# gaurav00700/Selfsupervised-NVSF

Hardware: AMD Instinct MI355X
Metric: rendered rays/sec (LiDAR+cam) (higher is better)
Workload: dtype f16; 1 GPU; C2: KITTI-360 seq-1908-shaped frame per GPU, uniform sampling, static hash field; num_rays=4096, num_rays_lidar=4096, num_steps=768, hash_grid=L16 F2 T2^19 base16 max2048, sigma_mlp=32-64-16, heads=lidar 2x(87-64-64-1), rgb 31-64-64-3, parallelism=frame-sharded x1, no collective

## Files before the change

selfsupervised-nvsf_amd/csrc/common.h:

```cpp
#pragma once
#include <hip/hip_runtime.h>
#include <stdint.h>

#define NVSF_API extern "C" __attribute__((visibility("default")))

enum : int {
    NVSF_OK = 0,
    NVSF_ERR_INVALID_ARG = -1,
    NVSF_ERR_UNSUPPORTED = -2,
};

constexpr int kWave = 64;

static inline int nvsf_launch_status() {
    hipError_t e = hipGetLastError();
    return e == hipSuccess ? NVSF_OK : (int)e;
}

static inline unsigned cdiv(unsigned long long a, unsigned b) { return (unsigned)((a + b - 1) / b); }

enum NvsfVariantKey : int {
    kVarMarch = 0,
    kVarPlanesFwd,
    kVarPlanesBwd,
    kVarHashgridFwd,
    kVarHashgridBwd,
    kVarHash4dBwd,
    kVarSlicePlan,
    kVarRenderTail,
    kVarMarchSkew,
    kVarMlpBwd,
    kVarLevelKinds,
    kVarCount
};
int nvsf_variant(int key);
int nvsf_cu_count();

__device__ __forceinline__ int lane_id() { return (int)(threadIdx.x & 63); }

template <typename T>
__device__ __forceinline__ T wave_sum(T v) {
#pragma unroll
    for (int o = 32; o > 0; o >>= 1) v += __shfl_xor(v, o, 64);
    return v;
}

__device__ __forceinline__ float wave_scan_add(float v) {
    const int l = lane_id();
#pragma unroll
    for (int o = 1; o < 64; o <<= 1) {
        float u = __shfl_up(v, o, 64);
        if (l >= o) v += u;
    }
    return v;
}
__device__ __forceinline__ float wave_scan_mul(float v) {
    const int l = lane_id();
#pragma unroll
    for (int o = 1; o < 64; o <<= 1) {
        float u = __shfl_up(v, o, 64);
        if (l >= o) v *= u;
    }
    return v;
}
__device__ __forceinline__ uint32_t wave_scan_add_u32(uint32_t v) {
// ... 25 lines not shown
```

selfsupervised-nvsf_amd/csrc/fused_field.hip:

```cpp
#include "hashgrid_device.h"
#include "mlp_device.h"
#include "encodings_device.h"
#include "march_device.h"
#pragma clang diagnostic ignored "-Wpass-failed"
#include <stdlib.h>

namespace {
constexpr int kBlock = 256;
constexpr int kWavesPerBlock = kBlock / kWave;

struct RayBatch {
    const float* rays_o;
    const float* rays_d;
    const float* nears;
    const float* fars;
    const float* lin;
    const float* noise;
    float lo[3], hi[3];
    float inv_extent;
    float bound;
    uint32_t N, T;
};

template <int F>
// ... 68 lines not shown
__device__ __forceinline__ void fma_entry(float w, uint32_t raw, float& a0, float& a1) {
    asm("v_fma_mix_f32 %0, %1, %2, %0 op_sel_hi:[0,1,0]" : "+v"(a0) : "v"(w), "v"(raw));
    asm("v_fma_mix_f32 %0, %1, %2, %0 op_sel:[0,1,0] op_sel_hi:[0,1,0]" : "+v"(a1) : "v"(w), "v"(raw));
}

template <int F>
__device__ __forceinline__ uint32_t gather_raw(__amdgpu_buffer_rsrc_t rsrc, uint32_t byte_off);
template <>
__device__ __forceinline__ uint32_t gather_raw<2>(__amdgpu_buffer_rsrc_t rsrc, uint32_t byte_off) {
    return __builtin_amdgcn_raw_buffer_load_b32(rsrc, byte_off, 0, 0);
}
typedef uint32_t entry4_t __attribute__((ext_vector_type(2)));
template <int F> struct EntryOf { typedef uint32_t type; };
template <> struct EntryOf<4> { typedef entry4_t type; };
template <>
__device__ __forceinline__ uint32_t gather_raw<4>(__amdgpu_buffer_rsrc_t, uint32_t) = delete;
__device__ __forceinline__ entry4_t gather_raw4(__amdgpu_buffer_rsrc_t rsrc, uint32_t byte_off) {
    return __builtin_amdgcn_raw_buffer_load_b64(rsrc, byte_off, 0, 0);
}

template <int F>
struct DensityCtx {
    static constexpr int Q = 8 / F;
    LaneLevels<F> lv;
    half8_t w0[kHidTiles];
    OutLayerW wout;
    __amdgpu_buffer_rsrc_t rsrc;
    uint32_t first_hashed;
    int g;
    const uint4* lds_lv;
};

constexpr uint32_t kFirstHashedC2 = 5;
template <int F, int QG, bool LDS_LV = false, int FH = -1>
__device__ __forceinline__ half8_t density_encode(const DensityCtx<F>& cx, const float (&x)[3]) {
    constexpr int Q = 8 / F;
    LaneLevels<F> lv_local;
    if constexpr (LDS_LV) {
        uint32_t again = 0;
        asm volatile("" : "+v"(again));
#pragma unroll
        for (int q = 0; q < Q; ++q) {
            const uint4 v = cx.lds_lv[4 * q + again];
            lv_local.scale[q] = __builtin_bit_cast(float, v.x);
            lv_local.res[q] = v.y;
            lv_local.res2[q] = v.y * v.y;
            lv_local.boff[q] = v.z;
            lv_local.rows[q] = v.w;
        }
    }
    const LaneLevels<F>& lv = LDS_LV ? lv_local : cx.lv;
    const uint32_t first_hashed = FH >= 0 ? (uint32_t)FH : cx.first_hashed;
    const int g = cx.g;
    half8_t xf;
#pragma unroll
    for (int q0 = 0; q0 < Q; q0 += QG) {
    float frac[Q][3];
    typename EntryOf<F>::type raw[Q][8];
#pragma unroll
    for (int q = q0; q < q0 + QG; ++q) {
        uint32_t c[3];
#pragma unroll
        for (int d = 0; d < 3; ++d) {
            const float pos = fmaf(lv.scale[q], x[d], 0.5f);
            const float fl = floorf(pos);
            frac[q][d] = pos - fl;
            c[d] = (uint32_t)(int32_t)fl;
        }
        uint32_t idx[8];
        const bool all_dense = (uint32_t)(4 * q + 3) < first_hashed, all_hashed = (uint32_t)(4 * q) >= first_hashed;
        if (all_dense || !all_hashed) {
            const uint32_t b00 = c[0] + c[1] * lv.res[q] + c[2] * lv.res2[q];
            const uint32_t b10 = b00 + lv.res[q], b01 = b00 + lv.res2[q], b11 = b10 + lv.res2[q];
            const uint32_t base[4] = {b00, b10, b01, b11};
#pragma unroll
            for (int k = 0; k < 8; ++k) {
                uint32_t v = base[k >> 1] + (uint32_t)(k & 1);
                v = v >= lv.rows[q] ? v - lv.rows[q] : v;
                idx[k] = v;
            }
        }
        if (all_hashed || !all_dense) {
            const uint32_t hy0 = c[1] * 2654435761u, hy1 = hy0 + 2654435761u;
            const uint32_t hz0 = c[2] * 805459861u, hz1 = hz0 + 805459861u;
            const uint32_t yz[4] = {hy0 ^ hz0, hy1 ^ hz0, hy0 ^ hz1, hy1 ^ hz1};
            const uint32_t mask = lv.rows[q] - 1u;
            const bool lane_hashed = (uint32_t)(4 * q + g) >= first_hashed;
#pragma unroll
            for (int k = 0; k < 8; ++k) {
                const uint32_t v = ((c[0] + (uint32_t)(k & 1)) ^ yz[k >> 1]) & mask;
                idx[k] = (all_hashed || lane_hashed) ? v : idx[k];
            }
        }
#pragma unroll
        for (int k = 0; k < 8; ++k) {
            if constexpr (F == 2) raw[q][k] = gather_raw<2>(cx.rsrc, lv.boff[q] + idx[k] * (uint32_t)(F * sizeof(_Float16)));
            else raw[q][k] = gather_raw4(cx.rsrc, lv.boff[q] + idx[k] * (uint32_t)(F * sizeof(_Float16)));
        }
    }
#pragma unroll
    for (int q = q0; q < q0 + QG; ++q) {
        const float fx = frac[q][0], fy = frac[q][1], fz = frac[q][2];
        const float wx[2] = {1.0f - fx, fx}, wy[2] = {1.0f - fy, fy}, wz[2] = {1.0f - fz, fz};
        if constexpr (F == 2) {
            float a0 = 0.0f, a1 = 0.0f;
#pragma unroll
            for (int k = 0; k < 8; ++k) {
                const float w = (wx[k & 1] * wy[(k >> 1) & 1]) * wz[k >> 2];
                fma_entry(w, raw[q][k], a0, a1);
            }
            xf[q * F] = (_Float16)a0;
            xf[q * F + 1] = (_Float16)a1;
        } else {
            float a0 = 0.0f, a1 = 0.0f, a2 = 0.0f, a3 = 0.0f;
#pragma unroll
            for (int k = 0; k < 8; ++k) {
                const float w = (wx[k & 1] * wy[(k >> 1) & 1]) * wz[k >> 2];
                fma_entry(w, raw[q][k][0], a0, a1);
                fma_entry(w, raw[q][k][1], a2, a3);
            }
            xf[q * F] = (_Float16)a0;
            xf[q * F + 1] = (_Float16)a1;
            xf[q * F + 2] = (_Float16)a2;
            xf[q * F + 3] = (_Float16)a3;
        }
    }
    }
    return xf;
}

template <int F, int QG>
__device__ __forceinline__ float4_t density_eval(const DensityCtx<F>& cx, const float (&x)[3]) {
    const half8_t xf = density_encode<F, QG>(cx, x);
    float4_t acc1[kHidTiles];
#pragma unroll
    for (int t = 0; t < kHidTiles; ++t) {
        const float4_t zero = {0, 0, 0, 0};
        acc1[t] = mfma16(cx.w0[t], xf, zero);
    }
    half8_t h[kHidSteps];
    pack_hidden(acc1, h);
    return cx.wout.apply(h);
}

struct TrainOut {
    float* x01;
    _Float16* feat;
    float* h32;
    uint32_t* tile;
};

__device__ __forceinline__ void store_h32(float* __restrict__ h32, unsigned long long s, int lane, int g, float o0, float o1, float o2, float o3, bool ok) {
    const int from = (lane + 48) & 63;
    const float prev = __int_as_float(__builtin_amdgcn_ds_bpermute(from << 2, __float_as_int(o3)));
    if (ok) *reinterpret_cast<float4*>(h32 + s * 16 + 4 * g) = make_float4(prev, o0, o1, o2);
}

constexpr int kTrPitch = 20;
constexpr int kTrWords = 16 * kTrPitch;
// ... 1238 lines not shown
                    img[1] += w0 * cr[1];
                }
            } else {
                if (g == 0 && on) {
#pragma unroll
                    for (int k = 0; k < 3; ++k) {
                        cr[k] = sigmoid_f32(oa[k]);
                        img[k] += w0 * cr[k];
                    }
                }
            }
        }
        if constexpr (TRAIN) {
            if (g == 0 && valid) {
#pragma unroll
                for (int k = 0; k < C; ++k) rt.rgb[s * C + k] = cr[k];
            }
        }
    }
    ws = wave_sum(ws);
    dp = wave_sum(dp);
#pragma unroll
    for (int k = 0; k < C; ++k) img[k] = wave_sum(img[k]);
    if (lane == 0) {
        weights_sum[n] = ws;
        depth[n] = dp;
        const float bg[3] = {bg0, bg1, bg2};
        const float rest = use_bg ? 1.0f - ws : 0.0f;
#pragma unroll
        for (int k = 0; k < C; ++k) image[(size_t)n * C + k] = use_bg ? img[k] + rest * bg[k] : img[k];
    }
}

template <bool LIDAR, bool TRAIN = false>
__global__ __launch_bounds__(kBlock) __attribute__((amdgpu_waves_per_eu(4, 4))) void k_render_tail2(
    RayBatch rb, const uint2* __restrict__ feat, const _Float16* __restrict__ w_sigma, const _Float16* __restrict__ w_a,
    const _Float16* __restrict__ w_b, float k_scale, float w_thresh, float bg0, float bg1, float bg2, int use_bg,
    const float* __restrict__ z_vals, float* __restrict__ weights, float* __restrict__ weights_sum, float* __restrict__ depth,
    float* __restrict__ image, RenderTrainOut rt = RenderTrainOut()) {
    using FR = OccFrags<LIDAR>;
    constexpr int IN_STEPS = FR::IN_STEPS;
    constexpr int C = LIDAR ? 2 : 3;
    constexpr int kOut1 = FR::kCount;
    __shared__ half8_t s_frag[(FR::kCount + kHidSteps) * kWave];
    __shared__ float4_t s_pre[kWavesPerBlock * FR::kPre];
    const int lane = lane_id(), g = lane >> 4, c = lane & 15;
    for (int f = (int)(threadIdx.x >> 6); f < FR::kCount + kHidSteps; f += kWavesPerBlock)
        s_frag[f * kWave + lane] = f < FR::kCount ? occ_fragment<LIDAR>(f, lane, w_sigma, w_a, w_b) : load_w_chained(w_sigma + kHidden * 32, 0, f - FR::kCount, lane, 5);
    __syncthreads();
    const uint32_t n = __builtin_amdgcn_readfirstlane(blockIdx.x * kWavesPerBlock + (threadIdx.x >> 6));
    if (n >= rb.N) return;
    const half8_t* frag = s_frag + lane;
    const uint32_t T = rb.T;
    const size_t M = (size_t)rb.N * T;

    const float rd0 = rb.rays_d[3 * (size_t)n], rd1 = rb.rays_d[3 * (size_t)n + 1], rd2 = rb.rays_d[3 * (size_t)n + 2];
    const float d0 = (rd0 + 1.0f) / 2.0f, d1 = (rd1 + 1.0f) / 2.0f, d2 = (rd2 + 1.0f) / 2.0f;
    half8_t xf[IN_STEPS];
    if constexpr (!LIDAR) {
        float sh[16];
        sh4_basis(d0, d1, d2, sh);
#pragma unroll
        for (int j = 0; j < 8; ++j) xf[0][j] = (_Float16)(g == 0 ? sh[j] : sh[8 + j]);
    } else {
#pragma unroll
        for (int s = 0; s < 3; ++s)
#pragma unroll
            for (int j = 0; j < 8; j += 2) {
                const int k = 32 * s + 8 * g + j;
                float sn = 1.0f, cs = 1.0f;
                if (k < 72) {
                    const int i = k / 24, f = (k - 24 * i) >> 1;
                    freq_pair(i == 0 ? d0 : (i == 1 ? d1 : d2), f, sn, cs);
                }
                xf[s][j] = (_Float16)sn;
                xf[s][j + 1] = (_Float16)cs;
            }
    }
    const bool takes_geo = LIDAR ? (g == 1 || g == 2) : (g >= 2);
    const int src_a = (c + 16 * (LIDAR ? 2 * (g - 1) : 2 * (g - 2))) & 63, src_b = (src_a + 16) & 63;
    const int src_a1 = (src_a + 48) & 63, src_b1 = (src_b + 48) & 63;
    float4_t* pre = s_pre + (threadIdx.x >> 6) * FR::kPre;
    ray_head_constants<LIDAR>(xf, w_a, w_b, lane, pre);
    auto head2 = [&](int hd, const half8_t (&x_last)[2], float4_t (&out)[2]) {
        const int base = FR::kHead + hd * FR::kPerHead;
        float4_t acc[2][kHidTiles];
#pragma unroll
        for (int t = 0; t < kHidTiles; ++t) {
            float4_t c = {0, 0, 0, 0};
            if constexpr (IN_STEPS > 1) c = pre[(hd * 4 + t) * 4 + g];
            const half8_t w = frag[(base + t) * kWave];
            acc[0][t] = mfma16(w, x_last[0], c);
            acc[1][t] = mfma16(w, x_last[1], c);
        }
        half8_t h[2][kHidSteps];
        pack_hidden(acc[0], h[0]);
        pack_hidden(acc[1], h[1]);
#pragma unroll
        for (int t = 0; t < kHidTiles; ++t) {
            float4_t a0 = {0, 0, 0, 0}, a1 = {0, 0, 0, 0};
#pragma unroll
            for (int s = 0; s < kHidSteps; ++s) {
                const half8_t w = frag[(base + 4 + 2 * t + s) * kWave];
                a0 = mfma16(w, h[0][s], a0);
                a1 = mfma16(w, h[1][s], a1);
            }
            acc[0][t] = a0;
            acc[1][t] = a1;
        }
        pack_hidden(acc[0], h[0]);
        pack_hidden(acc[1], h[1]);
        float4_t a0 = {0, 0, 0, 0}, a1 = {0, 0, 0, 0};
#pragma unroll
        for (int s = 0; s < kHidSteps; ++s) {
            const half8_t w = frag[(base + 4 + 8 + s) * kWave];
            a0 = mfma16(w, h[0][s], a0);
            a1 = mfma16(w, h[1][s], a1);
        }
        out[0] = a0;
        out[1] = a1;
    };

    const float sample_dist = (rb.fars[n] - rb.nears[n]) / (float)T;
    const size_t row0 = (size_t)n * T;
    const uint2* plane0 = feat + (size_t)(2 * g) * M + row0;
    const uint2* plane1 = feat + (size_t)(2 * g + 1) * M + row0;
    const float* zrow = z_vals + row0;
    float carry = 1.0f, ws = 0.0f, dp = 0.0f, img[C];
#pragma unroll
    for (int k = 0; k < C; ++k) img[k] = 0.0f;
    typedef uint32_t u4_t __attribute__((ext_vector_type(4)));
    struct TileIn {
        uint2 p0, p1;
        float z;
    };
    auto fetch = [&](uint32_t i0, int u) {
        const uint32_t i = i0 + 16u * (uint32_t)u + (uint32_t)c;
        const uint32_t k = i < T ? i : T - 1u;
        TileIn t;
        t.p0 = plane0[k];
        t.p1 = plane1[k];
        t.z = zrow[k];
        return t;
    };
    TileIn cur[2] = {fetch(0, 0), fetch(0, 1)};
    for (uint32_t i0 = 0; i0 < T; i0 += 32) {
        const uint32_t j0 = i0 + 32u < T ? i0 + 32u : i0;
        const TileIn nxt[2] = {fetch(j0, 0), fetch(j0, 1)};
        bool valid[2];
        uint32_t idx[2];
        float z[2], z_next[2];
        half8_t feat8[2];
#pragma unroll
        for (int u = 0; u < 2; ++u) {
            const uint32_t i = i0 + 16u * u + (uint32_t)c;
            valid[u] = i < T;
            idx[u] = valid[u] ? i : T - 1u;
            z[u] = cur[u].z;
            const u4_t packed = {cur[u].p0.x, cur[u].p1.x, cur[u].p1.y, cur[u].p0.y};
            feat8[u] = __builtin_bit_cast(half8_t, packed);
            if constexpr (TRAIN)
                store_feat_row_swap(rt.feat, row0 + idx[u], g, make_uint4(packed.x, packed.y, packed.z, packed.w), valid[u]);
        }
        z_next[0] = row_shl1(row_first(z[1]), z[0]);
        z_next[1] = row_shl1(row_first(nxt[0].z), z[1]);
        float4_t o[2];
        {
            float4_t acc[2][kHidTiles];
#pragma unroll
            for (int tt = 0; tt < kHidTiles; ++tt) {
                const half8_t w = frag[(FR::kSigma + tt) * kWave];
                acc[0][tt] = mfma16(w, feat8[0], float4_t{0, 0, 0, 0});
                acc[1][tt] = mfma16(w, feat8[1], float4_t{0, 0, 0, 0});
            }
            half8_t h[2][kHidSteps];
            pack_hidden(acc[0], h[0]);
            pack_hidden(acc[1], h[1]);
            float4_t a0 = {0, 0, 0, 0}, a1 = {0, 0, 0, 0};
#pragma unroll
            for (int sx = 0; sx < kHidSteps; ++sx) {
                a0 = mfma16(frag[(FR::kSigma + 4 + sx) * kWave], h[0][sx], a0);
                a1 = mfma16(frag[(kOut1 + sx) * kWave], h[1][sx], a1);
            }
            o[0] = a0;
            o[1] = a1;
        }
        float w0[2];
        bool on[2];
        float w;
        {
            const bool hi = g == 3;
            const float lg = hi ? o[0][3] : o[1][3], zz = hi ? z[0] : z[1], zn = hi ? z_next[0] : z_next[1];
            const uint32_t i = i0 + (hi ? 0u : 16u) + (uint32_t)c;
            const bool live = g >= 2 && i < T;
            const float delta = (i + 1u < T) ? zn - zz : sample_dist;
            float alpha = 0.0f;
            if (live) alpha = 1.0f - expf(-delta * k_scale * expf(lg));
            const float om = live ? (1.0f - alpha + 1e-15f) : 1.0f;
            const float incl = row16_scan_mul(om);
            const float excl = row_shr<1>(1.0f, incl);
            const float carry1 = carry * readlane_f32(incl, 63);
            w = alpha * ((hi ? carry : carry1) * excl);
            carry = carry1 * readlane_f32(incl, 47);
            if (live) {
                weights[row0 + i] = w;
                if constexpr (TRAIN) rt.sigma[row0 + i] = expf(lg);
            }
            w0[0] = __shfl(w, 48 + c, 64);
            w0[1] = __shfl(w, 32 + c, 64);
            on[0] = w0[0] > w_thresh;
            on[1] = w0[1] > w_thresh;
            const float a0 = g == 0 ? w0[0] : 0.0f, a1 = g == 0 ? w0[1] : 0.0f;
            ws += a0;
            dp += a0 * z[0];
            ws += a1;
            dp += a1 * z[1];
        }
        float cr[2][C];
#pragma unroll
        for (int u = 0; u < 2; ++u)
#pragma unroll
            for (int k = 0; k < C; ++k) cr[u][k] = 0.0f;
        if constexpr (TRAIN) {
#pragma unroll
            for (int u = 0; u < 2; ++u) {
                const uint32_t q0 = pack_h2(o[u][0], o[u][1]), q1 = pack_h2(o[u][2], g == 3 - u ? 1.0f : o[u][3]);
                const int col = u ? 4 * ((g + 1) & 3) : 4 * g;
                if (valid[u]) *reinterpret_cast<uint2*>(rt.geo + (row0 + idx[u]) * 16 + col) = make_uint2(q0, q1);
            }
        }
        if (__ballot(w > w_thresh)) {
            half8_t x_last[2];
#pragma unroll
            for (int u = 0; u < 2; ++u) {
                const uint32_t p0 = pack_h2(o[u][0], o[u][1]), p1 = pack_h2(o[u][2], g == 3 - u ? 1.0f : o[u][3]);
                u4_t gv;
                gv[0] = (uint32_t)__shfl((int)p0, u ? src_a1 : src_a);
                gv[1] = (uint32_t)__shfl((int)p1, u ? src_a1 : src_a);
                gv[2] = (uint32_t)__shfl((int)p0, u ? src_b1 : src_b);
                gv[3] = (uint32_t)__shfl((int)p1, u ? src_b1 : src_b);
                x_last[u] = takes_geo ? __builtin_bit_cast(half8_t, gv) : xf[IN_STEPS - 1];
            }
            float4_t oa[2];
            head2(0, x_last, oa);
            if constexpr (LIDAR) {
                float4_t ob[2];
                head2(1, x_last, ob);
#pragma unroll
                for (int u = 0; u < 2; ++u)
                    if (g == 0 && on[u]) {
                        cr[u][0] = sigmoid_f32(oa[u][0]);
                        cr[u][1] = sigmoid_f32(ob[u][0]);
                        img[0] += w0[u] * cr[u][0];
                        img[1] += w0[u] * cr[u][1];
                    }
            } else {
#pragma unroll
                for (int u = 0; u < 2; ++u)
                    if (g == 0 && on[u]) {
#pragma unroll
                        for (int k = 0; k < 3; ++k) {
                            cr[u][k] = sigmoid_f32(oa[u][k]);
                            img[k] += w0[u] * cr[u][k];
                        }
                    }
            }
        }
        if constexpr (TRAIN) {
#pragma unroll
            for (int u = 0; u < 2; ++u)
                if (g == 0 && valid[u]) {
#pragma unroll
                    for (int k = 0; k < C; ++k) rt.rgb[(row0 + idx[u]) * C + k] = cr[u][k];
                }
        }
        cur[0] = nxt[0];
        cur[1] = nxt[1];
    }
    ws = wave_sum(ws);
    dp = wave_sum(dp);
#pragma unroll
    for (int k = 0; k < C; ++k) img[k] = wave_sum(img[k]);
    if (lane == 0) {
        weights_sum[n] = ws;
        depth[n] = dp;
        const float bg[3] = {bg0, bg1, bg2};
        const float rest = use_bg ? 1.0f - ws : 0.0f;
#pragma unroll
        for (int k = 0; k < C; ++k) image[(size_t)n * C + k] = use_bg ? img[k] + rest * bg[k] : img[k];
    }
}

int fill_meta(GridMeta& meta, uint32_t L, const float* scales, const uint32_t* res, const uint32_t* offsets) {
    if (L == 0 || L > (uint32_t)kMaxLevels || !scales || !res || !offsets) return NVSF_ERR_INVALID_ARG;
    for (uint32_t l = 0; l < L; ++l) {
        meta.scale[l] = scales[l];
        meta.res[l] = res[l];
        meta.offset[l] = offsets[l];
        if (offsets[l + 1] <= offsets[l] || res[l] == 0) return NVSF_ERR_INVALID_ARG;
    }
    meta.offset[L] = offsets[L];
    return NVSF_OK;
}
}

#define REQUIRE(cond) do { if (!(cond)) return NVSF_ERR_INVALID_ARG; } while (0)

static int density_uniform_impl(const float* rays_o, const float* rays_d, const float* nears, const float* fars,
                                const float* lin, const float* noise, const float* h_aabb, float bound, uint32_t N,
                                uint32_t T, const void* table_f16, uint32_t L, uint32_t F, const float* h_scales,
                                const uint32_t* h_res, const uint32_t* h_offsets, const void* sigma_weights_f16,
                                float* z_vals, float* sigmas, void* geo_f16, void* feat_scratch, uint32_t sliced_passes, hipStream_t stream,
                                const TrainOut* train = nullptr) {
    if (N == 0 || T == 0) return NVSF_OK;
    REQUIRE(rays_o && rays_d && nears && fars && lin && h_aabb && table_f16 && sigma_weights_f16 && z_vals && sigmas && geo_f16);
    REQUIRE(bound > 0.0f);
    REQUIRE((reinterpret_cast<uintptr_t>(table_f16) & 15u) == 0 && (reinterpret_cast<uintptr_t>(sigma_weights_f16) & 15u) == 0 &&
            (reinterpret_cast<uintptr_t>(geo_f16) & 15u) == 0);
    if (L * F != 32 || (F != 2 && F != 4)) return NVSF_ERR_UNSUPPORTED;
    GridMeta meta;
    const int st = fill_meta(meta, L, h_scales, h_res, h_offsets);
    if (st != NVSF_OK) return st;
    RayBatch rb;
// ... 237 lines not shown
    const _Float16* tb = reinterpret_cast<const _Float16*>(table_f16);
    const _Float16* ws = reinterpret_cast<const _Float16*>(sigma_weights_f16);
    const _Float16* wa = reinterpret_cast<const _Float16*>(head_a_weights_f16);
    const _Float16* wb = reinterpret_cast<const _Float16*>(head_b_weights_f16);
    const uint2* fp = reinterpret_cast<const uint2*>(feat_scratch);
    const float b0 = h_bg_color ? h_bg_color[0] : 0.0f, b1 = h_bg_color ? h_bg_color[1] : 0.0f, b2 = h_bg_color ? h_bg_color[2] : 0.0f;
    const int use_bg = (h_bg_color && !lidar) ? 1 : 0;
    const dim3 grid_dim(cdiv(N, kWavesPerBlock)), block(kBlock);
#define LAUNCH_RU_FH(LD, FF, FH)                                                                                                      \
    do {                                                                                                                              \
        if (train)                                                                                                                    \
            hipLaunchKernelGGL((k_render_uniform<LD, FF, true, FH>), grid_dim, block, 0, stream, rb, tb, (uint32_t)table_bytes, meta, \
                               first_hashed, fp, ws, wa, wb, k_scale, w_thresh, b0, b1, b2, use_bg, z_vals, weights, weights_sum,     \
                               depth, image, *train);                                                                                \
        else                                                                                                                          \
            hipLaunchKernelGGL((k_render_uniform<LD, FF, false, FH>), grid_dim, block, 0, stream, rb, tb, (uint32_t)table_bytes,      \
                               meta, first_hashed, fp, ws, wa, wb, k_scale, w_thresh, b0, b1, b2, use_bg, z_vals, weights,            \
                               weights_sum, depth, image, RenderTrainOut());                                                         \
    } while (0)
#define LAUNCH_RU(LD, FF)                                                                                                             \
    do {                                                                                                                              \
        if (!FF && first_hashed == kFirstHashedC2 && nvsf_variant(kVarLevelKinds) == 0) LAUNCH_RU_FH(LD, FF, (FF ? -1 : (int)kFirstHashedC2)); \
        else LAUNCH_RU_FH(LD, FF, -1);                                                                                                \
    } while (0)
#define LAUNCH_TAIL(LD)                                                                                                               \
    do {                                                                                                                              \
        if (train)                                                                                                                    \
            hipLaunchKernelGGL((k_render_tail2<LD, true>), grid_dim, block, 0, stream, rb, fp, ws, wa, wb, k_scale, w_thresh, b0, b1, \
                               b2, use_bg, z_vals, weights, weights_sum, depth, image, *train);                                      \
        else                                                                                                                          \
            hipLaunchKernelGGL((k_render_tail2<LD, false>), grid_dim, block, 0, stream, rb, fp, ws, wa, wb, k_scale, w_thresh, b0,    \
                               b1, b2, use_bg, z_vals, weights, weights_sum, depth, image, RenderTrainOut());                        \
    } while (0)
    const bool tail2 = nvsf_variant(kVarRenderTail) == 0;
    if (lidar) { if (fp) { if (tail2) LAUNCH_TAIL(true); else LAUNCH_RU(true, true); } else LAUNCH_RU(true, false); }
    else { if (fp) { if (tail2) LAUNCH_TAIL(false); else LAUNCH_RU(false, true); } else LAUNCH_RU(false, false); }
#undef LAUNCH_TAIL
#undef LAUNCH_RU
#undef LAUNCH_RU_FH
    return nvsf_launch_status();
}

NVSF_API int nvsf_render_uniform_fwd(const float* rays_o, const float* rays_d, const float* nears, const float* fars, const float* lin,
                                     const float* noise, const float* h_aabb, float bound, uint32_t N, uint32_t T, const void* table_f16,
                                     uint32_t L, uint32_t F, const float* h_scales, const uint32_t* h_res, const uint32_t* h_offsets,
                                     const void* sigma_weights_f16, int lidar, const void* head_a_weights_f16,
                                     const void* head_b_weights_f16, float k_scale, float w_thresh, const float* h_bg_color,
                                     const void* feat_scratch, float* z_vals, float* weights, float* weights_sum, float* depth, float* image,
                                     hipStream_t stream) {
    return render_uniform_impl(rays_o, rays_d, nears, fars, lin, noise, h_aabb, bound, N, T, table_f16, L, F, h_scales, h_res, h_offsets,
                               sigma_weights_f16, lidar, head_a_weights_f16, head_b_weights_f16, k_scale, w_thresh, h_bg_color, feat_scratch,
                               z_vals, weights, weights_sum, depth, image, stream, nullptr);
}

NVSF_API int nvsf_render_uniform_train_fwd(const float* rays_o, const float* rays_d, const float* nears, const float* fars, const float* lin,
                                           const float* noise, const float* h_aabb, float bound, uint32_t N, uint32_t T,
                                           const void* table_f16, uint32_t L, uint32_t F, const float* h_scales, const uint32_t* h_res,
                                           const uint32_t* h_offsets, const void* sigma_weights_f16, int lidar,
                                           const void* head_a_weights_f16, const void* head_b_weights_f16, float k_scale, float w_thresh,
                                           const float* h_bg_color, void* feat_scratch, float* z_vals, float* weights, float* weights_sum,
                                           float* depth, float* image, float* x01, void* feat_rows_f16, void* geo_f16, float* sigmas,
                                           float* rgbs, hipStream_t stream) {
    if (N == 0 || T == 0) return NVSF_OK;
    REQUIRE(x01 && feat_rows_f16 && geo_f16 && sigmas && rgbs && lin);
    REQUIRE((reinterpret_cast<uintptr_t>(feat_rows_f16) & 15u) == 0 && (reinterpret_cast<uintptr_t>(geo_f16) & 15u) == 0);
    RenderTrainOut rt;
    rt.x01 = x01; rt.feat = reinterpret_cast<_Float16*>(feat_rows_f16); rt.geo = reinterpret_cast<_Float16*>(geo_f16);
    rt.sigma = sigmas; rt.rgb = rgbs;
    if (feat_scratch) {
// ... 11 lines not shown
```

selfsupervised-nvsf_amd/csrc/version.hip:

```cpp
#include "common.h"
#include <string.h>
NVSF_API const char* nvsf_version(void) { return "nvsf_hip 0.1.0 gfx950"; }

#ifndef NVSF_CSRC_DIGEST_ALL
#define NVSF_CSRC_DIGEST_ALL "unknown_________"
#endif
#ifndef NVSF_CSRC_DIGEST_RENDER
#define NVSF_CSRC_DIGEST_RENDER "unknown_________"
#endif
#define NVSF_MARK_ALL "NVSF_CSRC_DIGEST_ALL="
#define NVSF_MARK_RENDER "NVSF_CSRC_DIGEST_RENDER="
static const char g_digest_all[] = NVSF_MARK_ALL NVSF_CSRC_DIGEST_ALL;
static const char g_digest_render[] = NVSF_MARK_RENDER NVSF_CSRC_DIGEST_RENDER;
NVSF_API const char* nvsf_build_digest(int which) {
    return which == 1 ? g_digest_render + sizeof(NVSF_MARK_RENDER) - 1 : g_digest_all + sizeof(NVSF_MARK_ALL) - 1;
}

static int g_variant[kVarCount] = {};
__attribute__((visibility("hidden"))) int nvsf_variant(int key) { return key >= 0 && key < kVarCount ? g_variant[key] : 0; }

__attribute__((visibility("hidden"))) int nvsf_cu_count() {
    static const int n = [] {
        int dev = 0, v = 0;
        if (hipGetDevice(&dev) != hipSuccess || hipDeviceGetAttribute(&v, hipDeviceAttributeMultiprocessorCount, dev) != hipSuccess || v <= 0) v = 256;
        return v;
    }();
    return n;
}

NVSF_API int nvsf_test_variant(const char* name, int value) {
    static const char* const names[kVarCount] = {"march", "planes_fwd", "planes_bwd", "hashgrid_fwd", "hashgrid_bwd", "hash4d_bwd", "slice_plan",
                                                 "render_tail", "march_skew", "mlp_bwd", "level_kinds"};
    if (!name || value < 0) return NVSF_ERR_INVALID_ARG;
    for (int k = 0; k < kVarCount; ++k)
        if (strcmp(name, names[k]) == 0) {
            const int old = g_variant[k];
            g_variant[k] = value;
            return old;
        }
    return NVSF_ERR_INVALID_ARG;
}
```

selfsupervised-nvsf_amd/nvsf/testing.py:

```python
import contextlib

_NATIVE = {
    "march": {"wave": 0, "thread": 1, "serial": 2},
    "planes_fwd": {"runs": 0, "sample": 1},
    "planes_bwd": {"runs": 0, "atomic": 1, "global": 2},
    "hashgrid_fwd": {"auto": 0, "generic": 1},
    "hashgrid_bwd": {"corners": 0, "atomic": 1},
    "hash4d_bwd": {"lds": 0, "runs": 1},
    "slice_plan": {"balanced": 0, "home": 1},
    "render_tail": {"two": 0, "one": 1},
    "mlp_bwd": {"auto": 0, "staged": 1, "wave": 2},
    "level_kinds": {"compiled": 0, "runtime": 1},
    "march_skew": {"off": 0, **{f"queue{q}": q + 1 for q in range(8)}},
}
_PYTHON = {
    "heads_input": ("prefix", "rows"),
    "density_sliced": (None, False, True),
    "hash4d_train": ("fused", "slices"),
    "dynamic_fused": (True, False),
    "density_tail_train": ("fused", "chain"),
    "density_fn": ("fused", "chain"),
    "planes_train": ("fused", "separate"),
    "density_grad": ("composed", "matrix"),
    "hash4d_scatter": ("side", "main"),
    "table_scatter": ("binned", "atomic"),
}
_state = {}


def get(name):
    return _state.get(name, _PYTHON[name][0])


@contextlib.contextmanager
def variant(**choices):
    from nvsf import _hip
    lib = _hip.load()
    undo_native, undo_python = [], []
    try:
        for name, value in choices.items():
            if name in _NATIVE:
                code = _NATIVE[name][value]
                old = lib.nvsf_test_variant(name.encode(), code)
# ... 17 lines not shown
```

Measured before the change: 12.84 million rays/s.

## Add paired-sample gather render kernel overlapping hash gathers with sigma MLP

After: 12.91 million rays/s (median of 6 runs). No clear change (+0.5%).

```diff
diff --git a/selfsupervised-nvsf_amd/csrc/common.h b/selfsupervised-nvsf_amd/csrc/common.h
--- a/selfsupervised-nvsf_amd/csrc/common.h
+++ b/selfsupervised-nvsf_amd/csrc/common.h
@@ -31,6 +31,7 @@
     kVarMarchSkew,
     kVarMlpBwd,
     kVarLevelKinds,
+    kVarRenderGather,
     kVarCount
 };
 int nvsf_variant(int key);
diff --git a/selfsupervised-nvsf_amd/csrc/fused_field.hip b/selfsupervised-nvsf_amd/csrc/fused_field.hip
--- a/selfsupervised-nvsf_amd/csrc/fused_field.hip
+++ b/selfsupervised-nvsf_amd/csrc/fused_field.hip
@@ -124,39 +124,46 @@
 };
 
 constexpr uint32_t kFirstHashedC2 = 5;
-template <int F, int QG, bool LDS_LV = false, int FH = -1>
-__device__ __forceinline__ half8_t density_encode(const DensityCtx<F>& cx, const float (&x)[3]) {
+template <int F, int QG>
+struct EncodeGathers {
+    float frac[QG][3];
+    typename EntryOf<F>::type raw[QG][8];
+};
+
+template <int F, bool LDS_LV>
+__device__ __forceinline__ void encode_levels(const DensityCtx<F>& cx, LaneLevels<F>& lv) {
     constexpr int Q = 8 / F;
-    LaneLevels<F> lv_local;
     if constexpr (LDS_LV) {
         uint32_t again = 0;
         asm volatile("" : "+v"(again));
 #pragma unroll
         for (int q = 0; q < Q; ++q) {
             const uint4 v = cx.lds_lv[4 * q + again];
-            lv_local.scale[q] = __builtin_bit_cast(float, v.x);
-            lv_local.res[q] = v.y;
-            lv_local.res2[q] = v.y * v.y;
-            lv_local.boff[q] = v.z;
-            lv_local.rows[q] = v.w;
-        }
-    }
-    const LaneLevels<F>& lv = LDS_LV ? lv_local : cx.lv;
+            lv.scale[q] = __builtin_bit_cast(float, v.x);
+            lv.res[q] = v.y;
+            lv.res2[q] = v.y * v.y;
+            lv.boff[q] = v.z;
+            lv.rows[q] = v.w;
+        }
+    } else {
+        lv = cx.lv;
+    }
+}
+
+template <int F, int QG, int FH>
+__device__ __forceinline__ void density_encode_issue(const DensityCtx<F>& cx, const LaneLevels<F>& lv, const float (&x)[3], int q0,
+                                                     EncodeGathers<F, QG>& eg) {
     const uint32_t first_hashed = FH >= 0 ? (uint32_t)FH : cx.first_hashed;
     const int g = cx.g;
-    half8_t xf;
-#pragma unroll
-    for (int q0 = 0; q0 < Q; q0 += QG) {
-    float frac[Q][3];
-    typename EntryOf<F>::type raw[Q][8];
-#pragma unroll
-    for (int q = q0; q < q0 + QG; ++q) {
+#pragma unroll
+    for (int r = 0; r < QG; ++r) {
+        const int q = q0 + r;
         uint32_t c[3];
 #pragma unroll
         for (int d = 0; d < 3; ++d) {
             const float pos = fmaf(lv.scale[q], x[d], 0.5f);
             const float fl = floorf(pos);
-            frac[q][d] = pos - fl;
+            eg.frac[r][d] = pos - fl;
             c[d] = (uint32_t)(int32_t)fl;
         }
         uint32_t idx[8];
@@ -186,20 +193,25 @@
         }
 #pragma unroll
         for (int k = 0; k < 8; ++k) {
-            if constexpr (F == 2) raw[q][k] = gather_raw<2>(cx.rsrc, lv.boff[q] + idx[k] * (uint32_t)(F * sizeof(_Float16)));
-            else raw[q][k] = gather_raw4(cx.rsrc, lv.boff[q] + idx[k] * (uint32_t)(F * sizeof(_Float16)));
-        }
-    }
-#pragma unroll
-    for (int q = q0; q < q0 + QG; ++q) {
-        const float fx = frac[q][0], fy = frac[q][1], fz = frac[q][2];
+            if constexpr (F == 2) eg.raw[r][k] = gather_raw<2>(cx.rsrc, lv.boff[q] + idx[k] * (uint32_t)(F * sizeof(_Float16)));
+            else eg.raw[r][k] = gather_raw4(cx.rsrc, lv.boff[q] + idx[k] * (uint32_t)(F * sizeof(_Float16)));
+        }
+    }
+}
+
+template <int F, int QG>
+__device__ __forceinline__ void density_encode_blend(const EncodeGathers<F, QG>& eg, int q0, half8_t& xf) {
+#pragma unroll
+    for (int r = 0; r < QG; ++r) {
+        const int q = q0 + r;
+        const float fx = eg.frac[r][0], fy = eg.frac[r][1], fz = eg.frac[r][2];
         const float wx[2] = {1.0f - fx, fx}, wy[2] = {1.0f - fy, fy}, wz[2] = {1.0f - fz, fz};
         if constexpr (F == 2) {
             float a0 = 0.0f, a1 = 0.0f;
 #pragma unroll
             for (int k = 0; k < 8; ++k) {
                 const float w = (wx[k & 1] * wy[(k >> 1) & 1]) * wz[k >> 2];
-                fma_entry(w, raw[q][k], a0, a1);
+                fma_entry(w, eg.raw[r][k], a0, a1);
             }
             xf[q * F] = (_Float16)a0;
             xf[q * F + 1] = (_Float16)a1;
@@ -208,8 +220,8 @@
 #pragma unroll
             for (int k = 0; k < 8; ++k) {
                 const float w = (wx[k & 1] * wy[(k >> 1) & 1]) * wz[k >> 2];
-                fma_entry(w, raw[q][k][0], a0, a1);
-                fma_entry(w, raw[q][k][1], a2, a3);
+                fma_entry(w, eg.raw[r][k][0], a0, a1);
+                fma_entry(w, eg.raw[r][k][1], a2, a3);
             }
             xf[q * F] = (_Float16)a0;
             xf[q * F + 1] = (_Float16)a1;
@@ -217,6 +229,19 @@
             xf[q * F + 3] = (_Float16)a3;
         }
     }
+}
+
+template <int F, int QG, bool LDS_LV = false, int FH = -1>
+__device__ __forceinline__ half8_t density_encode(const DensityCtx<F>& cx, const float (&x)[3]) {
+    constexpr int Q = 8 / F;
+    LaneLevels<F> lv;
+    encode_levels<F, LDS_LV>(cx, lv);
+    half8_t xf;
+#pragma unroll
+    for (int q0 = 0; q0 < Q; q0 += QG) {
+        EncodeGathers<F, QG> eg;
+        density_encode_issue<F, QG, FH>(cx, lv, x, q0, eg);
+        density_encode_blend<F, QG>(eg, q0, xf);
     }
     return xf;
 }
@@ -1521,31 +1546,8 @@
     }
 }
 
-template <bool LIDAR, bool TRAIN = false>
-__global__ __launch_bounds__(kBlock) __attribute__((amdgpu_waves_per_eu(4, 4))) void k_render_tail2(
-    RayBatch rb, const uint2* __restrict__ feat, const _Float16* __restrict__ w_sigma, const _Float16* __restrict__ w_a,
-    const _Float16* __restrict__ w_b, float k_scale, float w_thresh, float bg0, float bg1, float bg2, int use_bg,
-    const float* __restrict__ z_vals, float* __restrict__ weights, float* __restrict__ weights_sum, float* __restrict__ depth,
-    float* __restrict__ image, RenderTrainOut rt = RenderTrainOut()) {
-    using FR = OccFrags<LIDAR>;
-    constexpr int IN_STEPS = FR::IN_STEPS;
-    constexpr int C = LIDAR ? 2 : 3;
-    constexpr int kOut1 = FR::kCount;
-    __shared__ half8_t s_frag[(FR::kCount + kHidSteps) * kWave];
-    __shared__ float4_t s_pre[kWavesPerBlock * FR::kPre];
-    const int lane = lane_id(), g = lane >> 4, c = lane & 15;
-    for (int f = (int)(threadIdx.x >> 6); f < FR::kCount + kHidSteps; f += kWavesPerBlock)
-        s_frag[f * kWave + lane] = f < FR::kCount ? occ_fragment<LIDAR>(f, lane, w_sigma, w_a, w_b) : load_w_chained(w_sigma + kHidden * 32, 0, f - FR::kCount, lane, 5);
-    __syncthreads();
-    const uint32_t n = __builtin_amdgcn_readfirstlane(blockIdx.x * kWavesPerBlock + (threadIdx.x >> 6));
-    if (n >= rb.N) return;
-    const half8_t* frag = s_frag + lane;
-    const uint32_t T = rb.T;
-    const size_t M = (size_t)rb.N * T;
-
-    const float rd0 = rb.rays_d[3 * (size_t)n], rd1 = rb.rays_d[3 * (size_t)n + 1], rd2 = rb.rays_d[3 * (size_t)n + 2];
-    const float d0 = (rd0 + 1.0f) / 2.0f, d1 = (rd1 + 1.0f) / 2.0f, d2 = (rd2 + 1.0f) / 2.0f;
-    half8_t xf[IN_STEPS];
+template <bool LIDAR>
+__device__ __forceinline__ void ray_dir_fragments(float d0, float d1, float d2, int g, half8_t (&xf)[OccFrags<LIDAR>::IN_STEPS]) {
     if constexpr (!LIDAR) {
         float sh[16];
         sh4_basis(d0, d1, d2, sh);
@@ -1566,21 +1568,57 @@
                 xf[s][j + 1] = (_Float16)cs;
             }
     }
-    const bool takes_geo = LIDAR ? (g == 1 || g == 2) : (g >= 2);
-    const int src_a = (c + 16 * (LIDAR ? 2 * (g - 1) : 2 * (g - 2))) & 63, src_b = (src_a + 16) & 63;
-    const int src_a1 = (src_a + 48) & 63, src_b1 = (src_b + 48) & 63;
-    float4_t* pre = s_pre + (threadIdx.x >> 6) * FR::kPre;
-    ray_head_constants<LIDAR>(xf, w_a, w_b, lane, pre);
-    auto head2 = [&](int hd, const half8_t (&x_last)[2], float4_t (&out)[2]) {
+}
+
+template <bool LIDAR>
+struct PairTail {
+    using FR = OccFrags<LIDAR>;
+    static constexpr int IN_STEPS = FR::IN_STEPS;
+    static constexpr int C = LIDAR ? 2 : 3;
+    static constexpr int kOut1 = FR::kCount;
+    static constexpr int kFrags = FR::kCount + kHidSteps;
+    typedef uint32_t u4_t __attribute__((ext_vector_type(4)));
+
+    const half8_t* frag;
+    const float4_t* pre;
+    half8_t x_dir;
+    int g, c, src_a, src_b, src_a1, src_b1;
+    bool takes_geo;
+    uint32_t T;
+    size_t row0;
+    float sample_dist, k_scale, w_thresh;
+    float carry, ws, dp, img[C];
+
+    static __device__ __forceinline__ half8_t fragment(int f, int lane, const _Float16* __restrict__ w_sigma, const _Float16* __restrict__ w_a,
+                                                       const _Float16* __restrict__ w_b) {
+        return f < FR::kCount ? occ_fragment<LIDAR>(f, lane, w_sigma, w_a, w_b) : load_w_chained(w_sigma + kHidden * 32, 0, f - FR::kCount, lane, 5);
+    }
+
+    __device__ __forceinline__ void init(const half8_t* frag_, const float4_t* pre_, const half8_t& x_dir_, int lane, uint32_t T_, size_t row0_,
+                                         float sample_dist_, float k_scale_, float w_thresh_) {
+        frag = frag_; pre = pre_; x_dir = x_dir_;
+        g = lane >> 4; c = lane & 15;
+        takes_geo = LIDAR ? (g == 1 || g == 2) : (g >= 2);
+        src_a = (c + 16 * (LIDAR ? 2 * (g - 1) : 2 * (g - 2))) & 63;
+        src_b = (src_a + 16) & 63;
+        src_a1 = (src_a + 48) & 63;
+        src_b1 = (src_b + 48) & 63;
+        T = T_; row0 = row0_; sample_dist = sample_dist_; k_scale = k_scale_; w_thresh = w_thresh_;
+        carry = 1.0f; ws = 0.0f; dp = 0.0f;
+#pragma unroll
+        for (int k = 0; k < C; ++k) img[k] = 0.0f;
+    }
+
+    __device__ __forceinline__ void head2(int hd, const half8_t (&x_last)[2], float4_t (&out)[2]) const {
         const int base = FR::kHead + hd * FR::kPerHead;
         float4_t acc[2][kHidTiles];
 #pragma unroll
         for (int t = 0; t < kHidTiles; ++t) {
-            float4_t c = {0, 0, 0, 0};
-            if constexpr (IN_STEPS > 1) c = pre[(hd * 4 + t) * 4 + g];
+            float4_t c0 = {0, 0, 0, 0};
+            if constexpr (IN_STEPS > 1) c0 = pre[(hd * 4 + t) * 4 + g];
             const half8_t w = frag[(base + t) * kWave];
-            acc[0][t] = mfma16(w, x_last[0], c);
-            acc[1][t] = mfma16(w, x_last[1], c);
+            acc[0][t] = mfma16(w, x_last[0], c0);
+            acc[1][t] = mfma16(w, x_last[1], c0);
         }
         half8_t h[2][kHidSteps];
         pack_hidden(acc[0], h[0]);
@@ -1608,72 +1646,11 @@
         }
         out[0] = a0;
         out[1] = a1;
-    };
-
-    const float sample_dist = (rb.fars[n] - rb.nears[n]) / (float)T;
-    const size_t row0 = (size_t)n * T;
-    const uint2* plane0 = feat + (size_t)(2 * g) * M + row0;
-    const uint2* plane1 = feat + (size_t)(2 * g + 1) * M + row0;
-    const float* zrow = z_vals + row0;
-    float carry = 1.0f, ws = 0.0f, dp = 0.0f, img[C];
-#pragma unroll
-    for (int k = 0; k < C; ++k) img[k] = 0.0f;
-    typedef uint32_t u4_t __attribute__((ext_vector_type(4)));
-    struct TileIn {
-        uint2 p0, p1;
-        float z;
-    };
-    auto fetch = [&](uint32_t i0, int u) {
-        const uint32_t i = i0 + 16u * (uint32_t)u + (uint32_t)c;
-        const uint32_t k = i < T ? i : T - 1u;
-        TileIn t;
-        t.p0 = plane0[k];
-        t.p1 = plane1[k];
-        t.z = zrow[k];
-        return t;
-    };
-    TileIn cur[2] = {fetch(0, 0), fetch(0, 1)};
-    for (uint32_t i0 = 0; i0 < T; i0 += 32) {
-        const uint32_t j0 = i0 + 32u < T ? i0 + 32u : i0;
-        const TileIn nxt[2] = {fetch(j0, 0), fetch(j0, 1)};
-        bool valid[2];
-        uint32_t idx[2];
-        float z[2], z_next[2];
-        half8_t feat8[2];
-#pragma unroll
-        for (int u = 0; u < 2; ++u) {
-            const uint32_t i = i0 + 16u * u + (uint32_t)c;
-            valid[u] = i < T;
-            idx[u] = valid[u] ? i : T - 1u;
-            z[u] = cur[u].z;
-            const u4_t packed = {cur[u].p0.x, cur[u].p1.x, cur[u].p1.y, cur[u].p0.y};
-            feat8[u] = __builtin_bit_cast(half8_t, packed);
-            if constexpr (TRAIN)
-                store_feat_row_swap(rt.feat, row0 + idx[u], g, make_uint4(packed.x, packed.y, packed.z, packed.w), valid[u]);
-        }
-        z_next[0] = row_shl1(row_first(z[1]), z[0]);
-        z_next[1] = row_shl1(row_first(nxt[0].z), z[1]);
-        float4_t o[2];
-        {
-            float4_t acc[2][kHidTiles];
-#pragma unroll
-            for (int tt = 0; tt < kHidTiles; ++tt) {
-                const half8_t w = frag[(FR::kSigma + tt) * kWave];
-                acc[0][tt] = mfma16(w, feat8[0], float4_t{0, 0, 0, 0});
-                acc[1][tt] = mfma16(w, feat8[1], float4_t{0, 0, 0, 0});
-            }
-            half8_t h[2][kHidSteps];
-            pack_hidden(acc[0], h[0]);
-            pack_hidden(acc[1], h[1]);
-            float4_t a0 = {0, 0, 0, 0}, a1 = {0, 0, 0, 0};
-#pragma unroll
-            for (int sx = 0; sx < kHidSteps; ++sx) {
-                a0 = mfma16(frag[(FR::kSigma + 4 + sx) * kWave], h[0][sx], a0);
-                a1 = mfma16(frag[(kOut1 + sx) * kWave], h[1][sx], a1);
-            }
-            o[0] = a0;
-            o[1] = a1;
-        }
+    }
+
+    template <bool TRAIN, bool STORE_Z>
+    __device__ __forceinline__ void pair(uint32_t i0, const float4_t (&o)[2], const float (&z)[2], const float (&z_next)[2], float* __restrict__ weights,
+                                         float* __restrict__ z_out, const RenderTrainOut& rt) {
         float w0[2];
         bool on[2];
         float w;
@@ -1693,6 +1670,7 @@
             carry = carry1 * readlane_f32(incl, 47);
             if (live) {
                 weights[row0 + i] = w;
+                if constexpr (STORE_Z) z_out[row0 + i] = zz;
                 if constexpr (TRAIN) rt.sigma[row0 + i] = expf(lg);
             }
             w0[0] = __shfl(w, 48 + c, 64);
@@ -1705,6 +1683,14 @@
             ws += a1;
             dp += a1 * z[1];
         }
+        bool valid[2];
+        uint32_t idx[2];
+#pragma unroll
+        for (int u = 0; u < 2; ++u) {
+            const uint32_t i = i0 + 16u * u + (uint32_t)c;
+            valid[u] = i < T;
+            idx[u] = valid[u] ? i : T - 1u;
+        }
         float cr[2][C];
 #pragma unroll
         for (int u = 0; u < 2; ++u)
@@ -1728,7 +1714,7 @@
                 gv[1] = (uint32_t)__shfl((int)p1, u ? src_a1 : src_a);
                 gv[2] = (uint32_t)__shfl((int)p0, u ? src_b1 : src_b);
                 gv[3] = (uint32_t)__shfl((int)p1, u ? src_b1 : src_b);
-                x_last[u] = takes_geo ? __builtin_bit_cast(half8_t, gv) : xf[IN_STEPS - 1];
+                x_last[u] = takes_geo ? __builtin_bit_cast(half8_t, gv) : x_dir;
             }
             float4_t oa[2];
             head2(0, x_last, oa);
@@ -1763,21 +1749,230 @@
                     for (int k = 0; k < C; ++k) rt.rgb[(row0 + idx[u]) * C + k] = cr[u][k];
                 }
         }
+    }
+
+    __device__ __forceinline__ void finish(int lane, uint32_t n, float bg0, float bg1, float bg2, int use_bg, float* __restrict__ weights_sum,
+                                           float* __restrict__ depth, float* __restrict__ image) {
+        ws = wave_sum(ws);
+        dp = wave_sum(dp);
+#pragma unroll
+        for (int k = 0; k < C; ++k) img[k] = wave_sum(img[k]);
+        if (lane == 0) {
+            weights_sum[n] = ws;
+            depth[n] = dp;
+            const float bg[3] = {bg0, bg1, bg2};
+            const float rest = use_bg ? 1.0f - ws : 0.0f;
+#pragma unroll
+            for (int k = 0; k < C; ++k) image[(size_t)n * C + k] = use_bg ? img[k] + rest * bg[k] : img[k];
+        }
+    }
+};
+
+template <bool LIDAR, bool TRAIN = false>
+__global__ __launch_bounds__(kBlock) __attribute__((amdgpu_waves_per_eu(4, 4))) void k_render_tail2(
+    RayBatch rb, const uint2* __restrict__ feat, const _Float16* __restrict__ w_sigma, const _Float16* __restrict__ w_a,
+    const _Float16* __restrict__ w_b, float k_scale, float w_thresh, float bg0, float bg1, float bg2, int use_bg,
+    const float* __restrict__ z_vals, float* __restrict__ weights, float* __restrict__ weights_sum, float* __restrict__ depth,
+    float* __restrict__ image, RenderTrainOut rt = RenderTrainOut()) {
+    using FR = OccFrags<LIDAR>;
+    using PT = PairTail<LIDAR>;
+    constexpr int IN_STEPS = FR::IN_STEPS;
+    __shared__ half8_t s_frag[PT::kFrags * kWave];
+    __shared__ float4_t s_pre[kWavesPerBlock * FR::kPre];
+    const int lane = lane_id(), g = lane >> 4, c = lane & 15;
+    for (int f = (int)(threadIdx.x >> 6); f < PT::kFrags; f += kWavesPerBlock) s_frag[f * kWave + lane] = PT::fragment(f, lane, w_sigma, w_a, w_b);
+    __syncthreads();
+    const uint32_t n = __builtin_amdgcn_readfirstlane(blockIdx.x * kWavesPerBlock + (threadIdx.x >> 6));
+    if (n >= rb.N) return;
+    const half8_t* frag = s_frag + lane;
+    const uint32_t T = rb.T;
+    const size_t M = (size_t)rb.N * T;
+
+    const float rd0 = rb.rays_d[3 * (size_t)n], rd1 = rb.rays_d[3 * (size_t)n + 1], rd2 = rb.rays_d[3 * (size_t)n + 2];
+    half8_t xf[IN_STEPS];
+    ray_dir_fragments<LIDAR>((rd0 + 1.0f) / 2.0f, (rd1 + 1.0f) / 2.0f, (rd2 + 1.0f) / 2.0f, g, xf);
+    float4_t* pre = s_pre + (threadIdx.x >> 6) * FR::kPre;
+    ray_head_constants<LIDAR>(xf, w_a, w_b, lane, pre);
+
+    const size_t row0 = (size_t)n * T;
+    PT pt;
+    pt.init(frag, pre, xf[IN_STEPS - 1], lane, T, row0, (rb.fars[n] - rb.nears[n]) / (float)T, k_scale, w_thresh);
+    const uint2* plane0 = feat + (size_t)(2 * g) * M + row0;
+    const uint2* plane1 = feat + (size_t)(2 * g + 1) * M + row0;
+    const float* zrow = z_vals + row0;
+    typedef uint32_t u4_t __attribute__((ext_vector_type(4)));
+    struct TileIn {
+        uint2 p0, p1;
+        float z;
+    };
+    auto fetch = [&](uint32_t i0, int u) {
+        const uint32_t i = i0 + 16u * (uint32_t)u + (uint32_t)c;
+        const uint32_t k = i < T ? i : T - 1u;
+        TileIn t;
+        t.p0 = plane0[k];
+        t.p1 = plane1[k];
+        t.z = zrow[k];
+        return t;
+    };
+    TileIn cur[2] = {fetch(0, 0), fetch(0, 1)};
+    for (uint32_t i0 = 0; i0 < T; i0 += 32) {
+        const uint32_t j0 = i0 + 32u < T ? i0 + 32u : i0;
+        const TileIn nxt[2] = {fetch(j0, 0), fetch(j0, 1)};
+        float z[2], z_next[2];
+        half8_t feat8[2];
+#pragma unroll
+        for (int u = 0; u < 2; ++u) {
+            z[u] = cur[u].z;
+            const u4_t packed = {cur[u].p0.x, cur[u].p1.x, cur[u].p1.y, cur[u].p0.y};
+            feat8[u] = __builtin_bit_cast(half8_t, packed);
+            if constexpr (TRAIN) {
+                const uint32_t i = i0 + 16u * u + (uint32_t)c;
+                store_feat_row_swap(rt.feat, row0 + (i < T ? i : T - 1u), g, make_uint4(packed.x, packed.y, packed.z, packed.w), i < T);
+            }
+        }
+        z_next[0] = row_shl1(row_first(z[1]), z[0]);
+        z_next[1] = row_shl1(row_first(nxt[0].z), z[1]);
+        float4_t o[2];
+        {
+            float4_t acc[2][kHidTiles];
+#pragma unroll
+            for (int tt = 0; tt < kHidTiles; ++tt) {
+                const half8_t w = frag[(FR::kSigma + tt) * kWave];
+                acc[0][tt] = mfma16(w, feat8[0], float4_t{0, 0, 0, 0});
+                acc[1][tt] = mfma16(w, feat8[1], float4_t{0, 0, 0, 0});
+            }
+            half8_t h[2][kHidSteps];
+            pack_hidden(acc[0], h[0]);
+            pack_hidden(acc[1], h[1]);
+            float4_t a0 = {0, 0, 0, 0}, a1 = {0, 0, 0, 0};
+#pragma unroll
+            for (int sx = 0; sx < kHidSteps; ++sx) {
+                a0 = mfma16(frag[(FR::kSigma + 4 + sx) * kWave], h[0][sx], a0);
+                a1 = mfma16(frag[(PT::kOut1 + sx) * kWave], h[1][sx], a1);
+            }
+            o[0] = a0;
+            o[1] = a1;
+        }
+        pt.template pair<TRAIN, false>(i0, o, z, z_next, weights, nullptr, rt);
         cur[0] = nxt[0];
         cur[1] = nxt[1];
     }
-    ws = wave_sum(ws);
-    dp = wave_sum(dp);
-#pragma unroll
-    for (int k = 0; k < C; ++k) img[k] = wave_sum(img[k]);
-    if (lane == 0) {
-        weights_sum[n] = ws;
-        depth[n] = dp;
-        const float bg[3] = {bg0, bg1, bg2};
-        const float rest = use_bg ? 1.0f - ws : 0.0f;
-#pragma unroll
-        for (int k = 0; k < C; ++k) image[(size_t)n * C + k] = use_bg ? img[k] + rest * bg[k] : img[k];
-    }
+    pt.finish(lane, n, bg0, bg1, bg2, use_bg, weights_sum, depth, image);
+}
+
+template <bool LIDAR, int FH = -1>
+__global__ __launch_bounds__(kBlock) __attribute__((amdgpu_waves_per_eu(4, 4))) void k_render_gather2(
+    RayBatch rb, const _Float16* __restrict__ table, uint32_t table_bytes, GridMeta meta, uint32_t first_hashed,
+    const _Float16* __restrict__ w_sigma, const _Float16* __restrict__ w_a, const _Float16* __restrict__ w_b, float k_scale, float w_thresh,
+    float bg0, float bg1, float bg2, int use_bg, float* __restrict__ z_vals, float* __restrict__ weights, float* __restrict__ weights_sum,
+    float* __restrict__ depth, float* __restrict__ image) {
+    using FR = OccFrags<LIDAR>;
+    using PT = PairTail<LIDAR>;
+    constexpr int F = 2;
+    constexpr int IN_STEPS = FR::IN_STEPS;
+    __shared__ uint4 s_lv[kMaxLevels];
+    __shared__ half8_t s_frag[PT::kFrags * kWave];
+    __shared__ float4_t s_pre[kWavesPerBlock * FR::kPre];
+    if (threadIdx.x < kMaxLevels) {
+        const uint32_t l = threadIdx.x;
+        s_lv[l] = make_uint4(__builtin_bit_cast(uint32_t, meta.scale[l]), meta.res[l], meta.offset[l] * (uint32_t)(F * sizeof(_Float16)),
+                             meta.offset[l + 1] - meta.offset[l]);
+    }
+    const int lane = lane_id(), g = lane >> 4, c = lane & 15;
+    for (int f = (int)(threadIdx.x >> 6); f < PT::kFrags; f += kWavesPerBlock) s_frag[f * kWave + lane] = PT::fragment(f, lane, w_sigma, w_a, w_b);
+    __syncthreads();
+    const uint32_t n = __builtin_amdgcn_readfirstlane(blockIdx.x * kWavesPerBlock + (threadIdx.x >> 6));
+    if (n >= rb.N) return;
+    const half8_t* frag = s_frag + lane;
+    const uint32_t T = rb.T;
+
+    DensityCtx<F> cx;
+    cx.g = g;
+    cx.first_hashed = first_hashed;
+    cx.lds_lv = s_lv + g;
+    cx.rsrc = __builtin_amdgcn_make_buffer_rsrc(const_cast<_Float16*>(table), 0, (int)table_bytes, 0x00020000);
+    const float rd0 = rb.rays_d[3 * (size_t)n], rd1 = rb.rays_d[3 * (size_t)n + 1], rd2 = rb.rays_d[3 * (size_t)n + 2];
+    half8_t xf[IN_STEPS];
+    ray_dir_fragments<LIDAR>((rd0 + 1.0f) / 2.0f, (rd1 + 1.0f) / 2.0f, (rd2 + 1.0f) / 2.0f, g, xf);
+    float4_t* pre = s_pre + (threadIdx.x >> 6) * FR::kPre;
+    ray_head_constants<LIDAR>(xf, w_a, w_b, lane, pre);
+
+    const float near = rb.nears[n], range = rb.fars[n] - near;
+    const float sample_dist = range / (float)T;
+    const float ox = rb.rays_o[3 * (size_t)n], oy = rb.rays_o[3 * (size_t)n + 1], oz = rb.rays_o[3 * (size_t)n + 2];
+    const size_t row0 = (size_t)n * T;
+    PT pt;
+    pt.init(frag, pre, xf[IN_STEPS - 1], lane, T, row0, sample_dist, k_scale, w_thresh);
+    const bool jitter = rb.noise != nullptr;
+    const float* nz_row = jitter ? rb.noise + row0 : rb.lin;
+    struct PairIn {
+        float lin[2], nz[2], lin_nxt, nz_nxt;
+    };
+    auto request = [&](uint32_t i0) {
+        PairIn p;
+#pragma unroll
+        for (int u = 0; u < 2; ++u) {
+            const uint32_t i = i0 + 16u * (uint32_t)u + (uint32_t)c;
+            const uint32_t ic = i < T ? i : T - 1u;
+            p.lin[u] = rb.lin[ic];
+            p.nz[u] = nz_row[ic];
+            if (u == 1) {
+                const uint32_t in = ic + 1u < T ? ic + 1u : ic;
+                p.lin_nxt = rb.lin[in];
+                p.nz_nxt = nz_row[in];
+            }
+        }
+        return p;
+    };
+    auto position = [&](float z, float (&x)[3]) {
+        x[0] = (fminf(fmaxf(ox + rd0 * z, rb.lo[0]), rb.hi[0]) + rb.bound) * rb.inv_extent;
+        x[1] = (fminf(fmaxf(oy + rd1 * z, rb.lo[1]), rb.hi[1]) + rb.bound) * rb.inv_extent;
+        x[2] = (fminf(fmaxf(oz + rd2 * z, rb.lo[2]), rb.hi[2]) + rb.bound) * rb.inv_extent;
+    };
+    auto sigma_mlp = [&](const half8_t& feat8, int out_base) {
+        float4_t acc1[kHidTiles];
+#pragma unroll
+        for (int tt = 0; tt < kHidTiles; ++tt) acc1[tt] = mfma16(frag[(FR::kSigma + tt) * kWave], feat8, float4_t{0, 0, 0, 0});
+        half8_t h[kHidSteps];
+        pack_hidden(acc1, h);
+        float4_t a = {0, 0, 0, 0};
+#pragma unroll
+        for (int sx = 0; sx < kHidSteps; ++sx) a = mfma16(frag[(out_base + sx) * kWave], h[sx], a);
+        return a;
+    };
+    PairIn cur = request(0u);
+    for (uint32_t i0 = 0; i0 < T; i0 += 32) {
+        const uint32_t j0 = i0 + 32u < T ? i0 + 32u : i0;
+        float z[2], z_next[2];
+#pragma unroll
+        for (int u = 0; u < 2; ++u) {
+            z[u] = near + range * cur.lin[u];
+            if (jitter) z[u] = z[u] + (cur.nz[u] - 0.5f) * sample_dist;
+        }
+        z_next[1] = near + range * cur.lin_nxt;
+        if (jitter) z_next[1] = z_next[1] + (cur.nz_nxt - 0.5f) * sample_dist;
+        z_next[0] = row_shl1(row_first(z[1]), z[0]);
+        cur = request(j0);
+        LaneLevels<F> lv;
+        encode_levels<F, true>(cx, lv);
+        float4_t o[2];
+        half8_t feat8;
+        float x[3];
+        EncodeGathers<F, 4> eg;
+        position(z[0], x);
+        density_encode_issue<F, 4, FH>(cx, lv, x, 0, eg);
+        density_encode_blend<F, 4>(eg, 0, feat8);
+        position(z[1], x);
+        encode_levels<F, true>(cx, lv);
+        density_encode_issue<F, 4, FH>(cx, lv, x, 0, eg);
+        __builtin_amdgcn_sched_barrier(0);
+        o[0] = sigma_mlp(feat8, FR::kSigma + 4);
+        __builtin_amdgcn_sched_barrier(0);
+        density_encode_blend<F, 4>(eg, 0, feat8);
+        o[1] = sigma_mlp(feat8, PT::kOut1);
+        pt.template pair<false, true>(i0, o, z, z_next, weights, z_vals, RenderTrainOut());
+    }
+    pt.finish(lane, n, bg0, bg1, bg2, use_bg, weights_sum, depth, image);
 }
 
 int fill_meta(GridMeta& meta, uint32_t L, const float* scales, const uint32_t* res, const uint32_t* offsets) {
@@ -2081,9 +2276,20 @@
             hipLaunchKernelGGL((k_render_tail2<LD, false>), grid_dim, block, 0, stream, rb, fp, ws, wa, wb, k_scale, w_thresh, b0,    \
                                b1, b2, use_bg, z_vals, weights, weights_sum, depth, image, RenderTrainOut());                        \
     } while (0)
+#define LAUNCH_GATHER2_FH(LD, FH)                                                                                                     \
+    hipLaunchKernelGGL((k_render_gather2<LD, FH>), grid_dim, block, 0, stream, rb, tb, (uint32_t)table_bytes, meta, first_hashed, ws, \
+                       wa, wb, k_scale, w_thresh, b0, b1, b2, use_bg, z_vals, weights, weights_sum, depth, image)
+#define LAUNCH_GATHER2(LD)                                                                                                            \
+    do {                                                                                                                              \
+        if (first_hashed == kFirstHashedC2 && nvsf_variant(kVarLevelKinds) == 0) LAUNCH_GATHER2_FH(LD, (int)kFirstHashedC2);          \
+        else LAUNCH_GATHER2_FH(LD, -1);                                                                                               \
+    } while (0)
     const bool tail2 = nvsf_variant(kVarRenderTail) == 0;
-    if (lidar) { if (fp) { if (tail2) LAUNCH_TAIL(true); else LAUNCH_RU(true, true); } else LAUNCH_RU(true, false); }
-    else { if (fp) { if (tail2) LAUNCH_TAIL(false); else LAUNCH_RU(false, true); } else LAUNCH_RU(false, false); }
+    const bool gather2 = !train && nvsf_variant(kVarRenderGather) == 0;
+    if (lidar) { if (fp) { if (tail2) LAUNCH_TAIL(true); else LAUNCH_RU(true, true); } else if (gather2) LAUNCH_GATHER2(true); else LAUNCH_RU(true, false); }
+    else { if (fp) { if (tail2) LAUNCH_TAIL(false); else LAUNCH_RU(false, true); } else if (gather2) LAUNCH_GATHER2(false); else LAUNCH_RU(false, false); }
+#undef LAUNCH_GATHER2
+#undef LAUNCH_GATHER2_FH
 #undef LAUNCH_TAIL
 #undef LAUNCH_RU
 #undef LAUNCH_RU_FH
diff --git a/selfsupervised-nvsf_amd/csrc/version.hip b/selfsupervised-nvsf_amd/csrc/version.hip
--- a/selfsupervised-nvsf_amd/csrc/version.hip
+++ b/selfsupervised-nvsf_amd/csrc/version.hip
@@ -30,7 +30,7 @@
 
 NVSF_API int nvsf_test_variant(const char* name, int value) {
     static const char* const names[kVarCount] = {"march", "planes_fwd", "planes_bwd", "hashgrid_fwd", "hashgrid_bwd", "hash4d_bwd", "slice_plan",
-                                                 "render_tail", "march_skew", "mlp_bwd", "level_kinds"};
+                                                 "render_tail", "march_skew", "mlp_bwd", "level_kinds", "render_gather"};
     if (!name || value < 0) return NVSF_ERR_INVALID_ARG;
     for (int k = 0; k < kVarCount; ++k)
         if (strcmp(name, names[k]) == 0) {
diff --git a/selfsupervised-nvsf_amd/nvsf/testing.py b/selfsupervised-nvsf_amd/nvsf/testing.py
--- a/selfsupervised-nvsf_amd/nvsf/testing.py
+++ b/selfsupervised-nvsf_amd/nvsf/testing.py
@@ -9,6 +9,7 @@
     "hash4d_bwd": {"lds": 0, "runs": 1},
     "slice_plan": {"balanced": 0, "home": 1},
     "render_tail": {"two": 0, "one": 1},
+    "render_gather": {"two": 0, "one": 1},
     "mlp_bwd": {"auto": 0, "staged": 1, "wave": 2},
     "level_kinds": {"compiled": 0, "runtime": 1},
     "march_skew": {"off": 0, **{f"queue{q}": q + 1 for q in range(8)}},
```
